# Intel-HLS/GenomicsDB

Measured on AMD Instinct MI355X. Metric: combined-gVCF positions/sec, higher is better.
Workload: dtype u8/int32

## Files before the change

__graft_entry__.py:

```python
import os
import sys

ROOT = os.path.dirname(os.path.abspath(__file__))
sys.path.insert(0, ROOT)
sys.path.insert(0, os.path.join(ROOT, "tests"))


def build():
    from genomicsdb_amd import build as b
    lib = b.build_native(verbose=True)
    b.build_oracle()
    b.build_hostsim()
    b.build_hostsim_variants()
    b.build_hostsim_import()
    b.build_hostsim_inflate()
    b.build_hostsim_import_bcf()
    b.build_hostsim_import_csv()
    b.build_hostsim_dispatch()
    from genomicsdb_amd import synth
    synth.lib()
    import genomicsdb_amd
    from genomicsdb_amd import _lib
    L = _lib.lib()
    for s in _lib.SYMBOLS:
        getattr(L, s)
    print("built", lib)


def smoke():
    import helpers
    from golden_cases import CASES
    import genomicsdb_amd
    case = [c for c in CASES if c[0] == "t6_7_8_vcf_at_0"][0]
    name, callsets, vid, ov, golden, mode = case
    cells = helpers.cells_for(callsets, vid)
    q, pb = helpers.query_json(callsets, vid, ov, mode)
    want, _, _ = helpers.oracle_run(q, cells)
    s = genomicsdb_amd.GenomicsDBQueryStream(query_json=q, cells=cells, buffer_capacity=4096)
    got = s.read()
    s.close()
    assert got == want, "device output differs from the oracle"
    assert got == helpers.golden_text(golden)
    print("smoke ok: %d bytes, bit-exact vs oracle and reference golden" % len(got))


if __name__ == "__main__":
    build()
    if len(sys.argv) > 1 and sys.argv[1] == "smoke":
        smoke()
```

genomicsdb_amd/build.py:

```python
import os
import subprocess
import sys

PKG = os.path.dirname(os.path.abspath(__file__))
ROOT = os.path.dirname(PKG)
CSRC = os.path.join(PKG, "csrc")
OBJ = os.path.join(ROOT, "build", "obj")
LIB = os.path.join(PKG, "libgenomicsdb_amd.so")
TOOL = os.path.join(PKG, "gt_mpi_gather")
TOOLS = {"gt_mpi_gather": TOOL, "vcf2tiledb": os.path.join(PKG, "vcf2tiledb")}

SOURCES = [
    "kernels/gdb_pipeline.hip",
    "kernels/gdb_bgzf.hip",
    "kernels/gdb_import.hip",
    "kernels/gdb_inflate.hip",
    "host/vid_mapper.cc",
    "host/variant_query_config.cc",
    "host/combine_plan.cc",
    "host/fragment.cc",
    "host/reference_genome.cc",
    "host/vcf_importer.cc",
    "host/vcf_index.cc",
    "api/genomicsdb_bcf_generator.cc",
# ... 48 lines not shown
    return LIB


def build_jni(verbose=False):
    jh = os.environ.get("JAVA_HOME", "")
    inc = os.path.join(jh, "include") if jh else ""
    if inc and os.path.exists(os.path.join(inc, "jni.h")):
        incs = ["-I" + inc, "-I" + os.path.join(inc, "linux")]
    else:
        incs = ["-I" + os.path.join(CSRC, "jni", "stub")]
    out = os.path.join(PKG, "libtiledbgenomicsdb.so")
    src = os.path.join(CSRC, "jni", "jni_query_stream.cc")
    if _newer(out, [src, LIB, os.path.join(CSRC, "jni", "stub", "jni.h"), os.path.join(ROOT, "include", "genomicsdb_amd.h")]):
        cmd = ["g++", "-O2", "-std=c++17", "-fPIC", "-shared", "-Wall"] + incs + [src, "-o", out, "-L" + PKG, "-lgenomicsdb_amd", "-Wl,-rpath,$ORIGIN"]
        if verbose:
            print(" ".join(cmd), flush=True)
        subprocess.check_call(cmd)
    return out


def build_oracle():
    subprocess.check_call(["make", "-s", "-C", os.path.join(ROOT, "oracle")])
    return os.path.join(ROOT, "oracle", "liboracle_gvcf.so")


def build_hostsim():
    subprocess.check_call(["make", "-s", "-C", os.path.join(ROOT, "tests", "hostsim")])
    subprocess.check_call(["make", "-s", "-C", os.path.join(ROOT, "tests", "jni_harness")])
    subprocess.check_call(["make", "-s", "-C", os.path.join(ROOT, "tests", "compat")])


def build_hostsim_variants():
    subprocess.check_call(["make", "-s", "-C", os.path.join(ROOT, "tests", "hostsim_variants")])
    return os.path.join(ROOT, "tests", "hostsim_variants", "libhostsim_variants.so")


def build_hostsim_import():
    subprocess.check_call(["make", "-s", "-C", os.path.join(ROOT, "tests", "hostsim_import")])
    return os.path.join(ROOT, "tests", "hostsim_import", "libhostsim_import.so")


def build_hostsim_import_bcf():
    d = os.path.join(ROOT, "tests", "hostsim_import_bcf")
    subprocess.check_call(["make", "-s", "-C", d])
    return os.path.join(d, "libhostsim_import_bcf.so"), os.path.join(d, "malformed_bcf")


def build_hostsim_import_csv():
    d = os.path.join(ROOT, "tests", "hostsim_import_csv")
    subprocess.check_call(["make", "-s", "-C", d])
    return os.path.join(d, "libhostsim_import_csv.so"), os.path.join(d, "hostsim_import_csv_main")


def build_hostsim_inflate():
    subprocess.check_call(["make", "-s", "-C", os.path.join(ROOT, "tests", "hostsim_inflate")])
    return os.path.join(ROOT, "tests", "hostsim_inflate", "libhostsim_inflate.so")


def build_hostsim_dispatch():
    subprocess.check_call(["make", "-s", "-C", os.path.join(ROOT, "tests", "hostsim_dispatch")])
    return os.path.join(ROOT, "tests", "hostsim_dispatch", "libhostsim_dispatch.so")


if __name__ == "__main__":
    print(build_native(verbose=True))
    print(build_oracle())
```

genomicsdb_amd/csrc/core/gdb_core.hpp:

```cpp
#pragma once
#include "gdb_types.h"

#if defined(__HIP_DEVICE_COMPILE__)
#define GDB_FETCH_ADD_U64(p, v) atomicAdd((unsigned long long*)(p), (unsigned long long)(v))
#else
static inline unsigned long long gdb_fetch_add_u64(unsigned long long* p, unsigned long long v) { const unsigned long long o = *p; *p = o + v; return o; }
#define GDB_FETCH_ADD_U64(p, v) gdb_fetch_add_u64((unsigned long long*)(p), (unsigned long long)(v))
#endif

#define GDB_CF_REFBLOCK 1u
#define GDB_CF_DELETION 2u
#define GDB_CF_HAS_NR 4u
#define GDB_CF_HEAVY 8u
#define GDB_CF_IN_WINDOW 16u
#define GDB_CF_NALT(f) (((f) >> 8) & 0xFFu)
#define GDB_CF_PLOIDY(f) (((f) >> 16) & 0xFu)

#define GDB_RF_NON_REF_EXISTS 1u
#define GDB_RF_REMAPPING_NEEDED 2u
#define GDB_RF_SKIP_G_FIELDS 4u

#define GDB_IF_SPANNING 1u
#define GDB_IF_GT_OVERRIDE 2u
#define GDB_IF_NO_NR 4u
// ... 1454 lines not shown
      if (fd.length == GDB_VL_G && (num_merged - 1) > pl.max_diploid_alt_alleles) continue;
      if (fd.ndim == 2) { info_asa_sum(cx, k, f, num_merged, non_ref_exists, !ref_block_only, false, sink, any, err); continue; }
      if (fd.combine_op == GDB_OP_ELEMENT_WISE_SUM || fd.combine_op == GDB_OP_CONCATENATE) {
        if (fd.elem == GDB_ET_FLOAT) info_vector_combine<float>(cx, k, f, fd.combine_op, num_merged, non_ref_exists, !ref_block_only, sink, any, err);
        else info_vector_combine<int32_t>(cx, k, f, fd.combine_op, num_merged, non_ref_exists, !ref_block_only, sink, any, err);
        continue;
      }
      if (fd.elem == GDB_ET_FLOAT) {
        float v;
        if (!reduce_scalar<float>(cx, k, f, fd.combine_op, false, v, err, num_merged, non_ref_exists, !ref_block_only)) continue;
        if (any) sink.put(';');
        sink.write(cx.names.text + cx.names.field_name_off[f], cx.names.field_name_len[f]);
        sink.put('=');
        put_float(sink, v);
      } else {
        int32_t v;
        if (!reduce_scalar<int32_t>(cx, k, f, fd.combine_op, false, v, err, num_merged, non_ref_exists, !ref_block_only)) continue;
        if (any) sink.put(';');
        sink.write(cx.names.text + cx.names.field_name_off[f], cx.names.field_name_len[f]);
        sink.put('=');
        put_i32(sink, v);
      }
      any = true;
    }
    for (int i = 0; i < pl.n_histogram; ++i)
      info_asa_histogram(cx, k, pl.histogram_bin_field[i], pl.histogram_count_field[i], num_merged, non_ref_exists, !ref_block_only, false, sink, any, err);
    int32_t dp = cx.pc.dp_sum[k];
    if ((pl.f_DP >= 0 || pl.f_DP_FORMAT >= 0) && dp > 0 && !ref_block_only) {
      if (any) sink.put(';');
      const char t[] = "DP="; sink.write(t, 3); put_i32(sink, dp);
      any = true;
    }
    if (!any) sink.put('.');
  }
  if (fmt_mask) {
    sink.put('\t');
    bool first = true;
    for (int i = 0; i < pl.n_format; ++i) {
      if (!((fmt_mask >> i) & 1)) continue;
      if (!first) sink.put(':');
      first = false;
      int f = pl.format_field[i];
      if (f == pl.f_DP_FORMAT || f == pl.f_DP) { sink.put('D'); sink.put('P'); }
      else sink.write(cx.names.text + cx.names.field_name_off[f], cx.names.field_name_len[f]);
    }
  }
}

struct EntryCtx {
  FragmentView fr;
  CombinePlan pl;
  CellMeta cm;
  HeavyLists hl;
};
struct RecordInfo { int num_merged; uint32_t rflags; uint32_t fmt_mask; int64_t hbase, hend; };

template <class Sink> GDB_HD void put_int_vector(Sink& s, const int32_t* p, int n) {
  if (n == 0) { s.put('.'); return; }
  for (int j = 0; j < n; ++j) {
    if (p[j] == GDB_BCF_INT32_VECTOR_END) break;
    if (j) s.put(',');
    if (p[j] == GDB_BCF_INT32_MISSING) s.put('.'); else put_i32(s, p[j]);
  }
}
template <class Sink> GDB_HD void put_int_or_missing(Sink& s, bool has, int32_t v) {
  if (!has || v == GDB_BCF_INT32_MISSING) s.put('.'); else put_i32(s, v);
}

struct EntryMaps {
  int8_t* m2i;
  const int8_t* i2m;
  int nr_in;
  int n_in;
  int64_t inc;
  uint32_t cf;
  uint8_t iflag;
  bool remap, nr_exists;
  bool light;
  GDB_HD int lookup(int j) const {
    if (light) return j == 0 ? 0 : nr_in;
    const int v = m2i[j];
    return v >= 0 ? v : nr_in;
  }
};

#define GDB_FIELD_FN GDB_HD

GDB_FIELD_FN int32_t gt_merged_allele(const EntryCtx& cx, const RecordInfo& ri, const EntryMaps& em, int32_t a, int out_i) {
  int32_t m = -1;
  if (em.iflag & GDB_IF_GT_OVERRIDE) {
    const int ra = cx.hl.gt_override[GDB_MAX_PLOIDY * em.inc + (out_i < GDB_MAX_PLOIDY ? out_i : GDB_MAX_PLOIDY - 1)];
    if (ra == 0) m = 0;
    else if (ra == 2) m = ri.num_merged - 1;
    else { for (int q = 1; q < em.n_in; ++q) if (em.i2m && em.i2m[q] >= 0 && em.i2m[q] != ri.num_merged - 1) { m = em.i2m[q]; break; } }
  } else if (a == GDB_TILEDB_NULL_INT32 || a == -1 || a == GDB_BCF_INT32_MISSING) {
    m = -1;
  } else if (!em.remap) {
    m = a;
  } else {
    int8_t mm = -1;
    if (a >= 0 && a < em.n_in) mm = em.i2m ? em.i2m[a] : (a == 0 ? (int8_t)0 : ((em.nr_exists && a == 1) ? (int8_t)(ri.num_merged - 1) : (int8_t)-1));
    if (mm >= 0) m = mm;
    else if ((em.iflag & GDB_IF_SPANNING) && (em.iflag & GDB_IF_NO_NR)) m = -1;
    else m = em.nr_exists ? ri.num_merged - 1 : -1;
  }
  return m;
}
template <class Sink> GDB_FIELD_FN Sink emit_GT(Sink s, const EntryCtx& cx, const RecordInfo& ri, const EntryMaps& em, int64_t c) {
  const CombinePlan& pl = cx.pl;
  const int f = pl.f_GT;
  int n;
  const int32_t* g = cell_field<int32_t>(cx.fr, pl, f, c, n);
  const bool pp = pl.field[f].length == GDB_VL_PP;
  const int step = pp ? 2 : 1;
  int out_i = 0;
  for (int j = 0; j < n; j += step, ++out_i) {
    if (out_i) s.put((pp && g[j - 1] > 0) ? '|' : '/');
    const int32_t m = pl.produce_GT_field ? gt_merged_allele(cx, ri, em, g[j], out_i) : -1;
    if (m < 0) s.put('.'); else put_i32(s, m);
  }
  if (out_i == 0) s.put('.');
  return s;
}

template <class Sink> GDB_FIELD_FN Sink emit_chars(Sink s, const EntryCtx& cx, int f, int64_t c) {
  int n;
  const char* p = cell_field<char>(cx.fr, cx.pl, f, c, n);
  int len = 0;
  while (len < n && p[len]) ++len;
  if (n == 0) s.put('.');
  for (int j = 0; j < len; ++j) { const char ch = p[j]; s.put(ch == 0x07 ? '.' : ch); }
  return s;
}

template <class Sink, class T> GDB_FIELD_FN Sink emit_vector(Sink s, const T* p, int n, uint32_t* err) {
  if (n == 0) { s.put('.'); return s; }
  for (int j = 0; j < n; ++j) {
    if (elem_is_vector_end(p[j])) break;
    if (j) s.put(',');
    put_elem(s, p[j], err);
  }
  return s;
}

template <class Sink, class T> GDB_FIELD_FN Sink emit_remap_alleles(Sink s, const T* p, int n, const EntryMaps& em, int num_merged, bool alt_only, uint32_t* err) {
  const int length = alt_only ? num_merged - 1 : num_merged;
  if (length == 0) { s.put('.'); return s; }
  for (int j = 0; j < length; ++j) {
    if (j) s.put(',');
    const int aj = alt_only ? j + 1 : j;
    const int in_j = em.lookup(aj);
    const int idx = alt_only ? in_j - 1 : in_j;
    const bool has = in_j >= 0 && idx >= 0 && idx < n;
    T v;
    if (has) v = p[idx]; else elem_set_missing(v);
    put_elem(s, v, err);
  }
  return s;
}

template <class Sink, class T> GDB_FIELD_FN Sink emit_remap_genotypes(Sink s, const T* p, int n, const EntryMaps& em, int num_merged, int ploidy, uint32_t* err) {
  if (ploidy == 1) {
    for (int j = 0; j < num_merged; ++j) {
      if (j) s.put(',');
      const int in_j = em.lookup(j);
      const bool has = in_j >= 0 && in_j < n;
      T v;
      if (has) v = p[in_j]; else elem_set_missing(v);
      put_elem(s, v, err);
    }
  } else if (ploidy == 2 && em.light) {
    T v3[3];
    uint64_t w3[3];
    int n3[3];
    const int nr = em.nr_in;
    for (int q = 0; q < 3; ++q) {
      const int gi = q == 0 ? 0 : q == 1 ? (nr >= 0 ? gdb_alleles2gt(0, nr) : -1) : (nr >= 0 ? gdb_alleles2gt(nr, nr) : -1);
      if (gi >= 0 && gi < n) v3[q] = p[gi]; else elem_set_missing(v3[q]);
      n3[q] = elem_pack_text(v3[q], w3[q]);
    }
    for (int kk = 0; kk < num_merged; ++kk)
      for (int j = 0; j <= kk; ++j) {
        const int q = kk == 0 ? 0 : (j == 0 ? 1 : 2);
        if (kk | j) s.put(',');
        if (n3[q]) put_packed(s, w3[q], n3[q]); else put_elem(s, v3[q], err);
      }
  } else if (ploidy == 2) {
    for (int kk = 0; kk < num_merged; ++kk) {
      const int in_k = em.lookup(kk);
      for (int j = 0; j <= kk; ++j) {
        if (kk | j) s.put(',');
        const int in_j = em.lookup(j);
        const bool both = in_j >= 0 && in_k >= 0;
        const int gi = both ? gdb_alleles2gt(in_j, in_k) : 0;
        const bool has = both && gi < n;
        T v;
        if (has) v = p[gi]; else elem_set_missing(v);
        put_elem(s, v, err);
      }
    }
  } else if (ploidy >= 3 && ploidy <= GDB_MAX_PLOIDY) {
    int g[GDB_MAX_PLOIDY], in[GDB_MAX_PLOIDY];
    for (int q = 0; q < ploidy; ++q) g[q] = 0;
    bool first = true;
    do {
      if (!first) s.put(',');
      first = false;
      bool missing = false;
      for (int q = 0; q < ploidy; ++q) { in[q] = em.lookup(g[q]); if (in[q] < 0) missing = true; }
      T v;
      elem_set_missing(v);
      if (!missing) { const int64_t gi = gdb_genotype_index(in, ploidy); if (gi < n) v = p[gi]; }
      put_elem(s, v, err);
    } while (gdb_next_genotype(g, ploidy, num_merged));
  } else {
    *err |= GDB_ERR_UNSUPPORTED_PLOIDY;
    s.put('.');
  }
  return s;
}

GDB_FIELD_FN void build_entry_maps(const EntryCtx& cx, const RecordInfo& ri, int64_t c, EntryMaps& em, int8_t* m2i_store, uint32_t* err) {
  em.m2i = m2i_store;
  em.remap = (ri.rflags & GDB_RF_REMAPPING_NEEDED) != 0;
  em.nr_exists = (ri.rflags & GDB_RF_NON_REF_EXISTS) != 0;
  em.nr_in = -1; em.i2m = nullptr; em.n_in = 0; em.iflag = 0; em.inc = -1; em.cf = 0; em.light = false;
  if (c < 0) return;
  em.cf = cx.cm.cflags[c];
  em.n_in = (int)GDB_CF_NALT(em.cf) + 1;
  if (!em.remap) return;
  if (!(em.cf & GDB_CF_HEAVY)) { em.light = true; em.nr_in = em.nr_exists ? 1 : -1; return; }
  for (int j = 0; j < ri.num_merged; ++j) em.m2i[j] = -1;
  if (em.cf & GDB_CF_HEAVY) {
    const int32_t row = cx.fr.row[c];
    int64_t lo = ri.hbase, hi = ri.hend;
    while (lo < hi) { int64_t mid = (lo + hi) >> 1; if (cx.fr.row[cx.hl.cell[mid]] < row) lo = mid + 1; else hi = mid; }
    if (lo < ri.hend && cx.hl.cell[lo] == c) em.inc = lo; else *err |= GDB_ERR_INTERNAL;
  }
  if (em.inc >= 0) {
    em.i2m = cx.hl.i2m + cx.hl.i2m_off[em.inc];
    em.iflag = cx.hl.iflags[em.inc];
    for (int a = 0; a < em.n_in; ++a) { const int8_t t = em.i2m[a]; if (t >= 0) em.m2i[t] = (int8_t)a; }
    if (em.nr_exists && (em.cf & GDB_CF_HAS_NR) && em.m2i[ri.num_merged - 1] >= 0) em.nr_in = em.m2i[ri.num_merged - 1];
  }
}

template <class Sink> GDB_HD Sink emit_field(Sink s, const EntryCtx& cx, const RecordInfo& ri, const EntryMaps& em, int i, int64_t c, uint32_t* err) {
  const CombinePlan& pl = cx.pl;
  const int f = pl.format_field[i];
  const GdbFieldDesc& fd = pl.field[f];
  if (f == pl.f_DP && pl.f_DP_FORMAT >= 0) {
    int32_t v = GDB_BCF_INT32_MISSING;
    if (field_valid(cx.cm, c, pl.f_DP_FORMAT)) { int n; const int32_t* p = cell_field<int32_t>(cx.fr, pl, pl.f_DP_FORMAT, c, n); if (n > 0) v = p[0]; }
    if (gdb_int_valid(v)) put_i32(s, v); else s.put('.');
  } else if (!field_valid(cx.cm, c, f)) {
    s.put('.');
  } else if (f == pl.f_GT) {
    s = emit_GT(s, cx, ri, em, c);
  } else if (fd.elem == GDB_ET_CHAR || fd.elem == GDB_ET_FLAG) {
    s = emit_chars(s, cx, f, c);
  } else if (fd.elem == GDB_ET_FLOAT) {
    int n;
    const float* p = cell_field<float>(cx.fr, pl, f, c, n);
    const bool allele_dep = fd.length == GDB_VL_A || fd.length == GDB_VL_R || fd.length == GDB_VL_G;
    if (!em.remap || !allele_dep) s = emit_vector(s, p, n, err);
    else if (fd.length == GDB_VL_G) s = emit_remap_genotypes(s, p, n, em, ri.num_merged, (int)GDB_CF_PLOIDY(em.cf), err);
    else s = emit_remap_alleles(s, p, n, em, ri.num_merged, fd.length == GDB_VL_A, err);
  } else if (fd.elem != GDB_ET_INT) {
    *err |= GDB_ERR_INTERNAL;
    s.put('.');
  } else {
    int n;
    const int32_t* p = cell_field<int32_t>(cx.fr, pl, f, c, n);
    const bool allele_dep = fd.length == GDB_VL_A || fd.length == GDB_VL_R || fd.length == GDB_VL_G;
    if (!em.remap || !allele_dep) s = emit_vector(s, p, n, err);
    else if (fd.length == GDB_VL_G) s = emit_remap_genotypes(s, p, n, em, ri.num_merged, (int)GDB_CF_PLOIDY(em.cf), err);
    else s = emit_remap_alleles(s, p, n, em, ri.num_merged, fd.length == GDB_VL_A, err);
  }
  return s;
}

template <class Sink> GDB_HD Sink entry_emit(const EntryCtx& cx, const RecordInfo& ri, int64_t c, Sink s, uint32_t* err) {
  const CombinePlan& pl = cx.pl;
  EntryMaps em;
  int8_t m2i_store[GDB_MAX_MERGED_ALLELES];
  build_entry_maps(cx, ri, c, em, m2i_store, err);
  bool first = true;
  for (int i = 0; i < pl.n_format; ++i) {
    if ((ri.fmt_mask >> i) & 1) {
      if (!first) s.put(':');
      first = false;
      if (c < 0) s.put('.');
      else s = emit_field(s, cx, ri, em, i, c, err);
    }
  }
  return s;
}
```

genomicsdb_amd/csrc/core/gdb_types.h:

```cpp
#pragma once
#include <stdint.h>

#if defined(__HIPCC__)
#define GDB_HD __host__ __device__ __forceinline__
#define GDB_HD_NOINLINE __host__ __device__
#else
#define GDB_HD inline
#define GDB_HD_NOINLINE
#endif

#define GDB_MAX_FIELDS 48
#define GDB_MAX_INFO_FIELDS 24
#define GDB_MAX_FORMAT_FIELDS 24
#define GDB_MAX_MERGED_ALLELES 128
#define GDB_MAX_INPUT_ALLELES 64
#define GDB_MAX_PLOIDY 8
#define GDB_MAX_INFO_VECTOR 64
#define GDB_MAX_ID_TOKENS 16
#define GDB_MAX_FILTER_IDS 16
#define GDB_MAX_PIPELINES_PER_PROCESS 256
#define GDB_MAX_HISTOGRAM_FIELDS 8

#define GDB_BCF_INT32_MISSING ((int32_t)0x80000000)
#define GDB_BCF_INT32_VECTOR_END ((int32_t)0x80000001)
// ... 21 lines not shown
  GDB_ERR_TOO_MANY_ID_TOKENS = 1u << 7,
  GDB_ERR_INFO_VECTOR_TOO_LONG = 1u << 8,
  GDB_ERR_CELL_STREAM = 1u << 9,
  GDB_ERR_TOO_MANY_FILTER_IDS = 1u << 10
};

struct GdbFieldDesc {
  int32_t elem;
  int32_t length;
  int32_t fixed_num;
  int32_t combine_op;
  int32_t is_info, is_format;
  int32_t known_enum;
  int32_t ndim;
  int32_t elem2d;
  int32_t delim0, delim1;
};

struct GdbColumn {
  const void* data;
  const uint32_t* off;
};

struct FragmentView {
  int64_t ncells;
  const int32_t* row;
  const int64_t* begin;
  const int64_t* end;
  GdbColumn col[GDB_MAX_FIELDS];
  int64_t nmarkers;
  const int64_t* marker_begin;
};

struct CombinePlan {
  int32_t nfields;
  GdbFieldDesc field[GDB_MAX_FIELDS];
  int32_t f_REF, f_ALT, f_GT, f_PL, f_DP, f_MIN_DP, f_DP_FORMAT, f_FILTER, f_QUAL, f_ID;
  int32_t n_info;
  int32_t info_field[GDB_MAX_INFO_FIELDS];
  int32_t n_histogram;
  int32_t histogram_bin_field[GDB_MAX_HISTOGRAM_FIELDS], histogram_count_field[GDB_MAX_HISTOGRAM_FIELDS];
  int32_t n_format;
  int32_t format_field[GDB_MAX_FORMAT_FIELDS];
  int32_t produce_GT_field, produce_FILTER_field, sites_only_query, min_PL_GT_for_spanning_deletions;
  int32_t max_diploid_alt_alleles;
  int32_t id_order_unordered_set;
  int32_t qual_combine_op;
  int32_t num_query_rows;
  int32_t bcf_mode;
  int32_t use_missing_values_not_vector_end;
  int32_t bcf_n_sample;
  int32_t bcf_end_id, bcf_dp_id;
  int32_t bcf_id[GDB_MAX_FIELDS];
};

struct GdbContig { int64_t offset, length; int32_t name_off, name_len; int32_t rid, pad; };

struct QueryWindow {
  int64_t qb, qe;
  const int32_t* row_to_qrow;
  int32_t num_array_rows;
  const GdbContig* contigs;
  int32_t ncontigs;
  const char* contig_names;
  const char* ref_bases;
  int64_t ref_begin, ref_len;
};
```

genomicsdb_amd/csrc/host/combine_plan.cc:

```cpp
#include "combine_plan.h"

#include <algorithm>
#include <array>
#include <map>
#include <unordered_map>
#include <cstring>
#include <set>

namespace genomicsdb_amd {

std::string HostPlan::bcf_header_bytes(bool keep_idx_fields) const {
  std::string text;
  for (size_t i = 0; i < header_lines.size(); ++i) {
    const std::string& l = header_lines[i];
    if (keep_idx_fields && header_line_idx[i] >= 0 && !l.empty() && l.back() == '>') text += l.substr(0, l.size() - 1) + ",IDX=" + std::to_string(header_line_idx[i]) + ">";
    else text += l;
    text += '\n';
  }
  text += header_text.substr(header_text.rfind("#CHROM"));
  std::string out("BCF\2\2", 5);
  const uint32_t l_text = (uint32_t)text.size() + 1;
  out.append((const char*)&l_text, 4);
  out += text;
  out.push_back('\0');
// ... 150 lines not shown
        throw UnsupportedOnDeviceException("INFO reducer on non-numeric field " + fi->m_name);
      if (pl.n_info >= GDB_MAX_INFO_FIELDS) throw UnsupportedOnDeviceException("too many INFO fields");
      pl.info_field[pl.n_info++] = f;
      add_field_to_hdr_if_missing(fi->m_vcf_name, 1);
    }
    if (add_FORMAT) {
      if (fi->m_is_vcf_FORMAT_field || op == GDB_OP_MOVE_TO_FORMAT) {
        if (fi->is_length_allele_dependent() && fi->m_element_type != GDB_ET_INT && fi->m_element_type != GDB_ET_FLOAT)
          throw UnsupportedOnDeviceException("allele-dependent non-numeric FORMAT field " + fi->m_name);
        fmt_list.push_back(f);
        add_field_to_hdr_if_missing(fi->m_vcf_name, 2);
      } else {
        dp_info_plan_field = f;
        add_field_to_hdr_if_missing("DP", 1);
      }
    }
  }
  for (auto& kv : histogram_pairs) {
    if (pl.n_histogram >= GDB_MAX_HISTOGRAM_FIELDS) throw UnsupportedOnDeviceException("too many histogram_sum fields");
    if (kv.second[0] < 0 || kv.second[1] < 0)
      throw BroadCombinedGVCFException("histogram_sum needs both tuple elements of field " + vid.get_field_info(kv.first).m_name + " among the queried attributes");
    pl.histogram_bin_field[pl.n_histogram] = kv.second[0];
    pl.histogram_count_field[pl.n_histogram] = kv.second[1];
    ++pl.n_histogram;
  }
  if (pl.f_FILTER >= 0)
    for (unsigned i = 0; i < vid.get_num_fields(); ++i) if (vid.get_field_info(i).m_is_vcf_FILTER_field) add_field_to_hdr_if_missing(vid.get_field_info(i).m_vcf_name, 0);
  if (!sites_only) {
    for (int f : fmt_list) if (f == pl.f_GT) pl.format_field[pl.n_format++] = f;
    for (int f : fmt_list) {
      if (f == pl.f_GT || f == pl.f_DP_FORMAT) continue;
      if (pl.n_format >= GDB_MAX_FORMAT_FIELDS - 1) throw UnsupportedOnDeviceException("too many FORMAT fields");
      pl.format_field[pl.n_format++] = f;
    }
    if (pl.f_DP_FORMAT >= 0 && (dp_info_plan_field >= 0 || std::find(fmt_list.begin(), fmt_list.end(), pl.f_DP_FORMAT) != fmt_list.end()))
      pl.format_field[pl.n_format++] = dp_info_plan_field >= 0 ? dp_info_plan_field : pl.f_DP_FORMAT;
  }
  if (dp_info_plan_field < 0 && pl.f_DP >= 0) {
    pl.f_DP = -1;
  }
  const FieldInfo* qual_info = vid.get_field_info("QUAL");
  if (qual_info && pl.f_QUAL >= 0 && qual_info->m_VCF_field_combine_operation != GDB_OP_UNKNOWN) {
    GdbCombineOp op = qual_info->m_VCF_field_combine_operation;
    if (op != GDB_OP_SUM && op != GDB_OP_MEAN && op != GDB_OP_MEDIAN) throw UnsupportedOnDeviceException("QUAL combine operation");
    pl.qual_combine_op = op;
  }
  pl.produce_GT_field = qc.produce_GT_field();
  pl.produce_FILTER_field = qc.produce_FILTER_field() && pl.f_FILTER >= 0;
  pl.sites_only_query = sites_only;
  pl.min_PL_GT_for_spanning_deletions = qc.produce_GT_with_min_PL_value_for_spanning_deletions();
  pl.max_diploid_alt_alleles = (int)qc.get_max_diploid_alt_alleles_that_can_be_genotyped();
  pl.id_order_unordered_set = qc.id_union_order_unordered_set() ? 1 : 0;
  pl.num_query_rows = (int)qc.get_num_rows_to_query();
  for (unsigned i = 0; i < vid.get_num_contigs(); ++i) {
    const ContigInfo& c = vid.get_contig_info(i);
    if (!hdr_contigs.count(c.m_name)) lines.push_back("##contig=<ID=" + c.m_name + ",length=" + std::to_string(c.m_length) + ">");
    GdbContig g;
    g.offset = c.m_tiledb_column_offset;
    g.length = c.m_length;
    g.name_off = (int32_t)hp.contig_names.size();
    g.name_len = (int32_t)c.m_name.size();
    hp.contig_names += c.m_name;
    hp.contigs.push_back(g);
  }
  {
    std::vector<std::pair<std::string, int>> dict;
    auto find_id = [&](const std::string& id) -> int { for (auto& d : dict) if (d.first == id) return d.second; return -1; };
    dict.push_back(std::make_pair(std::string("PASS"), 0));
    std::vector<std::pair<std::string, int>> ctg_dict;
    for (auto& l : lines) {
      int idx = -1;
      const bool is_dict = l.rfind("##FILTER=", 0) == 0 || l.rfind("##INFO=", 0) == 0 || l.rfind("##FORMAT=", 0) == 0;
      const bool is_ctg = l.rfind("##contig=", 0) == 0;
      size_t idp = l.find("<ID=");
      if ((is_dict || is_ctg) && idp != std::string::npos) {
        size_t ide = l.find_first_of(",>", idp + 4);
        const std::string id = l.substr(idp + 4, ide - idp - 4);
        if (is_dict) { idx = find_id(id); if (idx < 0) { idx = (int)dict.size(); dict.push_back(std::make_pair(id, idx)); } }
        else { idx = (int)ctg_dict.size(); ctg_dict.push_back(std::make_pair(id, idx)); }
      }
      hp.header_lines.push_back(l);
      hp.header_line_idx.push_back(idx);
    }
    for (int f = 0; f < GDB_MAX_FIELDS; ++f) pl.bcf_id[f] = -1;
    for (int f = 0; f < pl.nfields; ++f) { const FieldInfo* fi = vid.get_field_info(hp.field_names[(size_t)f]); if (fi) pl.bcf_id[f] = find_id(fi->m_vcf_name); }
    pl.bcf_end_id = find_id("END");
    pl.bcf_dp_id = find_id("DP");
    for (unsigned i = 0; i < vid.get_num_fields(); ++i) {
      const FieldInfo& fi = vid.get_field_info(i);
      hp.filter_bcf_id.push_back(have[0].count(fi.m_vcf_name) ? find_id(fi.m_vcf_name) : -1);
    }
    for (auto& g : hp.contigs) {
      const std::string name = hp.contig_names.substr((size_t)g.name_off, (size_t)g.name_len);
      g.rid = -1; g.pad = 0;
      for (auto& c : ctg_dict) if (c.first == name) g.rid = c.second;
    }
  }
  pl.bcf_mode = (output_format == "bu" || output_format == "b") ? 1 : 0;
  hp.bgzf = output_format == "z" || output_format == "b";
  if (!(output_format.empty() || output_format == "v" || output_format == "bu" || output_format == "z" || output_format == "b"))
    throw UnsupportedOnDeviceException("VCF output format \"" + output_format + "\": known formats are \"\" (VCF text), \"z\" (BGZF-compressed VCF), \"bu\" (BCF2) and \"b\" (BGZF-compressed BCF2)");
  pl.use_missing_values_not_vector_end = use_missing_values_not_vector_end ? 1 : 0;
  pl.bcf_n_sample = sites_only ? 0 : (int32_t)qc.get_num_rows_to_query();
  if (pl.bcf_mode && pl.bcf_end_id < 0) throw BroadCombinedGVCFException("BCF output needs an INFO END line in the header");
  std::sort(hp.contigs.begin(), hp.contigs.end(), [](const GdbContig& a, const GdbContig& b) { return a.offset < b.offset; });
  for (auto& l : lines) { hp.header_text += l; hp.header_text += '\n'; }
// ... 30 lines not shown
```

genomicsdb_amd/csrc/kernels/gdb_pipeline.hip:

```cpp
#include <hip/hip_runtime.h>

#include <fcntl.h>
#include <sys/stat.h>
#include <unistd.h>
#include <zlib.h>

#include <algorithm>
#include <cstdio>
#include <cstdlib>
#include <chrono>
#include <cstring>
#include <memory>
#include <mutex>
#include <thread>
#include <vector>

#include <rocprim/device/device_radix_sort.hpp>
#include <rocprim/device/device_reduce.hpp>
#include <rocprim/device/device_scan.hpp>
#include <rocprim/iterator/reverse_iterator.hpp>

#include "../core/gdb_stages.hpp"
#include "../core/gdb_bcf.hpp"
#include "../core/gdb_calls.hpp"
// ... 5040 lines not shown
      if ((fd.combine_op == GDB_OP_MEDIAN || fd.combine_op == GDB_OP_SUM || fd.combine_op == GDB_OP_MEAN) && (fd.elem == GDB_ET_FLOAT || fd.elem == GDB_ET_INT) && fd.length != GDB_VL_A)
        fields.push_back(std::make_pair(pl.info_field[i], 0));
    }
    if (pl.qual_combine_op != GDB_OP_UNKNOWN && pl.f_QUAL >= 0) fields.push_back(std::make_pair(pl.f_QUAL, 1));
    if (!fields.empty()) {
      S.scalar_pre.ensure(fields.size() * (size_t)T);
      for (size_t s = 0; s < fields.size(); ++s) {
        hipLaunchKernelGGL(k_scalar_values, dim3(blocks_for(T)), dim3(kBlock), 0, st, fr, pl, cm, rec, (const uint64_t*)S.inc_keys_sorted.p, (const int64_t*)S.inc_vals_sorted.p, T,
                           (int64_t)N, fields[s].first, fields[s].second, S.scalar_pre.p + s * (size_t)T);
        pre.slot[fields[s].first] = (int8_t)s;
      }
      pre.val = S.scalar_pre.p; pre.stride = T; pre.enabled = 1;
    }
  }
  HugeSites huge;
  memset(&huge, 0, sizeof(huge));
  SiteCtx sx0{fr, pl, cm, rec, hl, pc, nt, qw, so, med, big, tie, pre, huge};
  const int32_t huge_threshold = (P > 0 && T / P >= 24 && P <= (int64_t)kMaxHugeRecords) ? 24 : kHugeRecord;
  if (T > (int64_t)huge_threshold && !getenv("GDBAMD_NO_HUGE_SITES")) {
    S.huge_index.ensure((size_t)P); S.huge_list.ensure(kMaxHugeRecords); S.huge_out.ensure(kMaxHugeRecords); S.d_sx0.ensure(1);
    HIP_CHECK(hipMemcpyAsync(S.d_sx0.p, &sx0, sizeof(SiteCtx), hipMemcpyHostToDevice, st));
    STAGE("k_site_huge");
    hipLaunchKernelGGL(k_huge_records, dim3(blocks_for(P)), dim3(kBlock), 0, st, (const int64_t*)S.hbase.p, P, huge_threshold, S.huge_index.p, S.huge_list.p, S.counters.p + 3);
    hipLaunchKernelGGL(k_site_huge, dim3(1024), dim3(kHugeBlock), 0, st, (const SiteCtx*)S.d_sx0.p, (const int32_t*)S.huge_list.p, (const int32_t*)(S.counters.p + 3), S.huge_out.p, S.err.p);
    huge.index = S.huge_index.p; huge.out = S.huge_out.p; huge.enabled = 1;
  }
  SiteCtx sx{fr, pl, cm, rec, hl, pc, nt, qw, so, med, big, tie, pre, huge};
  S.d_sx.ensure(1);
  HIP_CHECK(hipMemcpyAsync(S.d_sx.p, &sx, sizeof(SiteCtx), hipMemcpyHostToDevice, st));
  STAGE("k_site_size");
  S.site_staging.ensure((size_t)P * kSiteStride + 64);
  S.spill_buf.ensure((size_t)P * kSpillTail); S.spill_chunk.ensure((size_t)P);
  const int32_t* site_order = nullptr;
  {
    static const bool sorted_sites = !(getenv("GDBAMD_SITE_ORDER") && atoi(getenv("GDBAMD_SITE_ORDER")) == 0);
    if (sorted_sites && P >= 4096) {
      S.site_key.ensure((size_t)P); S.site_key_sorted.ensure((size_t)P); S.site_ord_in.ensure((size_t)P); S.site_ord.ensure((size_t)P);
      hipLaunchKernelGGL(k_site_order_keys, dim3(blocks_for(P)), dim3(kBlock), 0, st, (const int64_t*)S.hbase.p, P, S.site_key.p, S.site_ord_in.p);
      S.sort_pairs(S.site_key.p, S.site_key_sorted.p, S.site_ord_in.p, S.site_ord.p, (size_t)P, 8);
      site_order = S.site_ord.p;
    }
  }
  hipLaunchKernelGGL(k_site_size, dim3(blocks_for(P, 64)), dim3(64), 0, st, S.d_sx.p, site_order, S.site_staging.p, SpillPool{S.spill_buf.p}, S.spill_chunk.p, S.err.p);
  S.remap_total.ensure(1);
  HIP_CHECK(hipMemsetAsync(S.remap_total.p, 0, sizeof(unsigned long long), st));
  for (int i = 0; i < pl.n_format; ++i)
    if (pl.format_field[i] == pl.f_PL && pl.f_PL >= 0)
      hipLaunchKernelGGL(k_remap_elements, dim3(blocks_for(P)), dim3(kBlock), 0, st, so, (const int32_t*)(d_fmt + (size_t)i * stride), P, i, S.remap_total.p);
  HIP_CHECK(hipEventRecord(ev[2], st));
  const int nchunks = (N + kAsmRows - 1) / kAsmRows;
  const size_t nchunk_total = (size_t)P * nchunks;
  S.chunk_size.ensure(nchunk_total + 1); S.chunk_off.ensure(nchunk_total + 2); S.rec_off.ensure(P + 2);
  RowIndex ri{S.row_ptr.p, S.perm.p, S.rm_begin.p};
  EntryCtx ex{fr, pl, cm, hl};
  HIP_CHECK(hipMemcpyToSymbolAsync(HIP_SYMBOL(c_ex), &ex, sizeof(EntryCtx), (size_t)S.ctx_slot * sizeof(EntryCtx), hipMemcpyHostToDevice, st));
  if (T >= (1ll << 32)) throw GenomicsDBDeviceException("more than 2^32 (record, variant call) incidences in one interval: split the query interval");
  S.type_hkeys.ensure(kTypeHash); S.type_hrep.ensure(kTypeHash); S.type_hid.ensure(kTypeHash); S.type_rep.ensure(kMaxTypes); S.rtype.ensure(P);
  HIP_CHECK(hipMemsetAsync(S.type_hkeys.p, 0xFF, kTypeHash * sizeof(unsigned long long), st));
  HIP_CHECK(hipMemsetAsync(S.type_hrep.p, 0x7F, kTypeHash * sizeof(int32_t), st));
  HIP_CHECK(hipMemsetAsync(S.type_hid.p, 0xFF, kTypeHash, st));
  HIP_CHECK(hipMemsetAsync(S.type_rep.p, 0, kMaxTypes * sizeof(int32_t), st));
  STAGE("k_type_insert");
  hipLaunchKernelGGL(k_type_insert, dim3(blocks_for(P)), dim3(kBlock), 0, st, so, P, S.type_hkeys.p, S.type_hrep.p);
  hipLaunchKernelGGL(k_type_assign, dim3(1), dim3(64), 0, st, S.type_hkeys.p, S.type_hrep.p, max_tabled_types(), S.type_hid.p, S.type_rep.p, S.counters.p + 1);
  S.untabled.ensure(P + 1); S.ubase.ensure(P + 1); S.urec.ensure(P + 1);
  hipLaunchKernelGGL(k_type_lookup, dim3(blocks_for(P)), dim3(kBlock), 0, st, so, P, S.type_hkeys.p, S.type_hid.p, S.rtype.p, S.untabled.p);
  S.excl_scan(S.untabled.p, S.ubase.p, (size_t)P);
  S.tmask.ensure(CW); S.nslots.ensure(CW + 1); S.tbase.ensure(CW + 1);
  STAGE("k_cell_types");
  {
    const size_t nocc = (size_t)kMaxTypes * (size_t)(P + 1);
    S.type_occ.ensure(nocc);
    HIP_CHECK(hipMemsetAsync(S.type_occ.p, 0, nocc * sizeof(uint32_t), st));
    hipLaunchKernelGGL(k_type_onehot, dim3(blocks_for(P)), dim3(kBlock), 0, st, (const uint8_t*)S.rtype.p, P, S.type_occ.p);
    S.excl_scan(S.type_occ.p, S.type_occ.p, nocc);
  }
  hipLaunchKernelGGL(k_cell_types, dim3(blocks_for(CW)), dim3(kBlock), 0, st, S.cflags.p, S.k_lo.p, S.k_hi.p, (const uint32_t*)S.type_occ.p, P,
                     (const int32_t*)(S.counters.p + 1), c_base, CW, S.tmask.p, S.nslots.p);
  S.excl_scan(S.nslots.p, S.tbase.p, (size_t)CW);
  uint32_t ur_a = 0, ur_b = 0, sl_a = 0, sl_b = 0;
  int32_t ntypes = 0;
  S.read_back_many({{&ur_a, S.ubase.p + (P - 1), 4}, {&ur_b, S.untabled.p + (P - 1), 4}, {&sl_a, S.tbase.p + (CW - 1), 4}, {&sl_b, S.nslots.p + (CW - 1), 4},
                    {&ntypes, S.counters.p + 1, 4}});
  const int64_t UR = (int64_t)ur_a + ur_b;
  const uint64_t SL = (uint64_t)sl_a + sl_b;
  if (UR > 0) hipLaunchKernelGGL(k_untabled_records, dim3(blocks_for(P)), dim3(kBlock), 0, st, S.untabled.p, S.ubase.p, P, S.urec.p);
  const uint64_t NS = (uint64_t)kMaxTypes + SL + (uint64_t)T + (uint64_t)UR * (uint64_t)N;
  if (NS >= (1ull << 32)) throw GenomicsDBDeviceException("entry text table exceeds 2^32 slots: split the query interval");
  S.slot_len.ensure(NS + 1); S.slot_units.ensure(NS + 1); S.slot_off.ensure(NS + 1); S.slot_desc.ensure(NS + 1);
  if (NS * (uint64_t)(kSlotStride / 16) >= (uint64_t)kOverflowBit) throw GenomicsDBDeviceException("entry text table exceeds 32 GiB: split the query interval");
  S.pool.ensure((size_t)NS * kSlotStride + 64);
  S.slot_bump.ensure(kBumpShards * 4);
  HIP_CHECK(hipMemsetAsync(S.slot_bump.p, 0, kBumpShards * 4 * sizeof(unsigned int), st));
  S.slot_over.ensure(kBumpShards);
  HIP_CHECK(hipMemsetAsync(S.slot_over.p, 0, kBumpShards * sizeof(unsigned int), st));
  bool wide = S.long_texts_seen;
  if (const char* e = getenv("GDBAMD_SLOT_STRIP")) wide = atoi(e) >= 256;
  auto shard_units_of = [&](size_t cap_bytes) { return (uint32_t)std::min<uint64_t>((uint64_t)(cap_bytes > 64 ? (cap_bytes - 64) / 16 : 0) / kBumpShards, ((uint64_t)kOverflowBit - 1) / kBumpShards); };
  if (wide) S.pool_ovf.ensure(std::max<size_t>((size_t)kBumpShards * ((size_t)S.pool_ovf_need * 16 + ((size_t)S.pool_ovf_need * 16 >> 3)), (size_t)1 << 20) + 64);
  SlotTable stt{S.slot_len.p, S.slot_off.p, S.pool.p, S.pool_ovf.p, (uint32_t)kMaxTypes, (uint32_t)(kMaxTypes + SL), (uint32_t)(kMaxTypes + SL + (uint64_t)T), S.slot_off.p, S.slot_bump.p,
                wide ? shard_units_of(S.pool_ovf.cap) : 0u, (int32_t)S.ctx_slot, pl.bcf_mode, pl.bcf_mode ? (uint32_t)kSlotStride : (uint32_t)kInlineText,
                (const int64_t*)S.hoff.p, (const int32_t*)S.k_lo.p, c_base, S.slot_over.p};
  STAGE("k_slots<0>");
#define GDB_SLOT_KERNELS(PASSN, W) do { \
  hipLaunchKernelGGL((k_slots_nocall<PASSN, W>), dim3(1), dim3(kMaxTypes), 0, st, stt, so, S.type_rep.p, ntypes, S.err.p); \
  if (SL > 0) hipLaunchKernelGGL((k_slots_light<PASSN, W>), dim3(blocks_for((int64_t)SL, light_block<W>())), dim3(light_block<W>()), 0, st, stt, so, S.type_rep.p, S.tmask.p, S.tbase.p, (const uint32_t*)S.slot_cell.p, c_base, (int64_t)SL, slot_regroup() ? 1 : 0, S.err.p); \
  if (T > 0) hipLaunchKernelGGL((k_slots_heavy<PASSN, W>), dim3(blocks_for(T, 64)), dim3(64), 0, st, stt, so, S.inc_keys_sorted.p, S.inc_vals_sorted.p, T, (int64_t)N, S.err.p); \
// ... 344 lines not shown
```

Measured before the change: 39.64 million.

## Add light-path per-cell FORMAT emitter driven by precomputed per-field op codes

```diff
diff --git a/__graft_entry__.py b/__graft_entry__.py
--- a/__graft_entry__.py
+++ b/__graft_entry__.py
@@ -17,6 +17,7 @@
     b.build_hostsim_import_bcf()
     b.build_hostsim_import_csv()
     b.build_hostsim_dispatch()
+    b.build_hostsim_light_emit()
     from genomicsdb_amd import synth
     synth.lib()
     import genomicsdb_amd
diff --git a/genomicsdb_amd/build.py b/genomicsdb_amd/build.py
--- a/genomicsdb_amd/build.py
+++ b/genomicsdb_amd/build.py
@@ -124,6 +124,12 @@
     return os.path.join(d, "libhostsim_import_csv.so"), os.path.join(d, "hostsim_import_csv_main")
 
 
+def build_hostsim_light_emit():
+    d = os.path.join(ROOT, "tests", "hostsim_light_emit")
+    subprocess.check_call(["make", "-s", "-C", d])
+    return os.path.join(d, "light_emit_diff"), os.path.join(d, "light_emit_diff_san")
+
+
 def build_hostsim_inflate():
     subprocess.check_call(["make", "-s", "-C", os.path.join(ROOT, "tests", "hostsim_inflate")])
     return os.path.join(ROOT, "tests", "hostsim_inflate", "libhostsim_inflate.so")
diff --git a/genomicsdb_amd/csrc/core/gdb_core.hpp b/genomicsdb_amd/csrc/core/gdb_core.hpp
--- a/genomicsdb_amd/csrc/core/gdb_core.hpp
+++ b/genomicsdb_amd/csrc/core/gdb_core.hpp
@@ -1530,6 +1530,7 @@
   CombinePlan pl;
   CellMeta cm;
   HeavyLists hl;
+  uint32_t generic_emit;
 };
 struct RecordInfo { int num_merged; uint32_t rflags; uint32_t fmt_mask; int64_t hbase, hend; };
 
@@ -1625,13 +1626,14 @@
   const int length = alt_only ? num_merged - 1 : num_merged;
   if (length == 0) { s.put('.'); return s; }
   for (int j = 0; j < length; ++j) {
-    if (j) s.put(',');
     const int aj = alt_only ? j + 1 : j;
     const int in_j = em.lookup(aj);
     const int idx = alt_only ? in_j - 1 : in_j;
     const bool has = in_j >= 0 && idx >= 0 && idx < n;
     T v;
     if (has) v = p[idx]; else elem_set_missing(v);
+    if (elem_is_vector_end(v)) break;
+    if (j) s.put(',');
     put_elem(s, v, err);
   }
   return s;
@@ -1640,11 +1642,12 @@
 template <class Sink, class T> GDB_FIELD_FN Sink emit_remap_genotypes(Sink s, const T* p, int n, const EntryMaps& em, int num_merged, int ploidy, uint32_t* err) {
   if (ploidy == 1) {
     for (int j = 0; j < num_merged; ++j) {
-      if (j) s.put(',');
       const int in_j = em.lookup(j);
       const bool has = in_j >= 0 && in_j < n;
       T v;
       if (has) v = p[in_j]; else elem_set_missing(v);
+      if (elem_is_vector_end(v)) break;
+      if (j) s.put(',');
       put_elem(s, v, err);
     }
   } else if (ploidy == 2 && em.light) {
@@ -1660,6 +1663,7 @@
     for (int kk = 0; kk < num_merged; ++kk)
       for (int j = 0; j <= kk; ++j) {
         const int q = kk == 0 ? 0 : (j == 0 ? 1 : 2);
+        if (elem_is_vector_end(v3[q])) return s;
         if (kk | j) s.put(',');
         if (n3[q]) put_packed(s, w3[q], n3[q]); else put_elem(s, v3[q], err);
       }
@@ -1667,13 +1671,14 @@
     for (int kk = 0; kk < num_merged; ++kk) {
       const int in_k = em.lookup(kk);
       for (int j = 0; j <= kk; ++j) {
-        if (kk | j) s.put(',');
         const int in_j = em.lookup(j);
         const bool both = in_j >= 0 && in_k >= 0;
         const int gi = both ? gdb_alleles2gt(in_j, in_k) : 0;
         const bool has = both && gi < n;
         T v;
         if (has) v = p[gi]; else elem_set_missing(v);
+        if (elem_is_vector_end(v)) return s;
+        if (kk | j) s.put(',');
         put_elem(s, v, err);
       }
     }
@@ -1682,13 +1687,14 @@
     for (int q = 0; q < ploidy; ++q) g[q] = 0;
     bool first = true;
     do {
-      if (!first) s.put(',');
-      first = false;
       bool missing = false;
       for (int q = 0; q < ploidy; ++q) { in[q] = em.lookup(g[q]); if (in[q] < 0) missing = true; }
       T v;
       elem_set_missing(v);
       if (!missing) { const int64_t gi = gdb_genotype_index(in, ploidy); if (gi < n) v = p[gi]; }
+      if (elem_is_vector_end(v)) break;
+      if (!first) s.put(',');
+      first = false;
       put_elem(s, v, err);
     } while (gdb_next_genotype(g, ploidy, num_merged));
   } else {
@@ -1730,7 +1736,7 @@
   if (f == pl.f_DP && pl.f_DP_FORMAT >= 0) {
     int32_t v = GDB_BCF_INT32_MISSING;
     if (field_valid(cx.cm, c, pl.f_DP_FORMAT)) { int n; const int32_t* p = cell_field<int32_t>(cx.fr, pl, pl.f_DP_FORMAT, c, n); if (n > 0) v = p[0]; }
-    if (gdb_int_valid(v)) put_i32(s, v); else s.put('.');
+    if (gdb_int_valid(v)) put_i32(s, v); else if (v != GDB_BCF_INT32_VECTOR_END) s.put('.');
   } else if (!field_valid(cx.cm, c, f)) {
     s.put('.');
   } else if (f == pl.f_GT) {
@@ -1758,8 +1764,133 @@
   return s;
 }
 
+GDB_HD int light_token(uint32_t sep, int32_t v, uint64_t& w) {
+  int n;
+  if (v == GDB_BCF_INT32_MISSING) { w = (uint64_t)'.'; n = 1; }
+  else if ((uint32_t)v < 100u) {
+    const uint32_t q = (uint32_t)v / 10u, r = (uint32_t)v - q * 10u;
+    w = q ? (uint64_t)(('0' + q) | (('0' + r) << 8)) : (uint64_t)('0' + r);
+    n = q ? 2 : 1;
+  }
+  else if ((uint32_t)v < 10000000u) w = gdb_pack_digits((uint32_t)v, n);
+  else return 0;
+  if (sep) { w = (w << 8) | (uint64_t)sep; ++n; }
+  return n;
+}
+template <class Sink> GDB_HD void put_token_w(Sink& s, uint64_t w, int n, uint32_t sep, int32_t v) {
+  if (n) put_packed(s, w, n);
+  else { if (sep) s.put((char)sep); put_i32(s, v); }
+}
+template <class Sink> GDB_HD void put_token(Sink& s, uint32_t sep, int32_t v) {
+  uint64_t w = 0;
+  const int n = light_token(sep, v, w);
+  put_token_w(s, w, n, sep, v);
+}
+template <class Sink> GDB_HD Sink entry_emit_light(const EntryCtx& cx, const RecordInfo& ri, int64_t c, uint32_t cf, uint64_t vmask, Sink s, uint32_t* err) {
+  const CombinePlan& pl = cx.pl;
+  const bool remap = (ri.rflags & GDB_RF_REMAPPING_NEEDED) != 0, nr_exists = (ri.rflags & GDB_RF_NON_REF_EXISTS) != 0;
+  const int nm = ri.num_merged;
+  const int nr_in = nr_exists ? 1 : -1;
+  uint32_t next_sep = 0;
+  for (int i = 0; i < pl.n_format; ++i) {
+    if (!((ri.fmt_mask >> i) & 1u)) continue;
+    const uint32_t sep = next_sep;
+    next_sep = ':';
+    const uint32_t op = pl.light_op[i];
+    const int f = (int)(op & 0xFFu);
+    uint32_t kind = (op >> 8) & 0xFu;
+    if (!((vmask >> f) & 1ull)) { put_token(s, sep, GDB_BCF_INT32_MISSING); continue; }
+    const GdbColumn& col = cx.fr.col[f];
+    int n;
+    const int32_t* p;
+    if (col.off) { const uint32_t a = col.off[c], b = col.off[c + 1]; n = (int)(b - a); p = (const int32_t*)col.data + a; }
+    else { n = (int)(op >> 12); p = (const int32_t*)col.data + c * n; }
+    if (kind >= GDB_LOP_R) {
+      if (!remap) kind = GDB_LOP_VEC;
+      else if (kind == GDB_LOP_G && GDB_CF_PLOIDY(cf) == 1u) kind = GDB_LOP_R;
+    }
+    switch (kind) {
+      case GDB_LOP_FIRST: {
+        const int32_t v = n > 0 ? p[0] : GDB_BCF_INT32_MISSING;
+        if (v != GDB_BCF_INT32_VECTOR_END) put_token(s, sep, v); else if (sep) s.put((char)sep);
+      } break;
+      case GDB_LOP_GT: case GDB_LOP_GT_PP: {
+        const bool pp = kind == GDB_LOP_GT_PP;
+        int out_i = 0;
+        for (int j = 0; j < n; j += pp ? 2 : 1, ++out_i) {
+          const uint32_t sp = out_i ? ((pp && p[j - 1] > 0) ? (uint32_t)'|' : (uint32_t)'/') : sep;
+          const int32_t a = p[j];
+          int32_t mg = GDB_BCF_INT32_MISSING;
+          if (pl.produce_GT_field && a != GDB_TILEDB_NULL_INT32 && a != -1 && a != GDB_BCF_INT32_MISSING) {
+            if (!remap) mg = a < 0 ? GDB_BCF_INT32_MISSING : a;
+            else mg = a == 0 ? 0 : (nr_exists ? nm - 1 : GDB_BCF_INT32_MISSING);
+          }
+          put_token(s, sp, mg);
+        }
+        if (out_i == 0) put_token(s, sep, GDB_BCF_INT32_MISSING);
+      } break;
+      case GDB_LOP_VEC: {
+        if (n == 0) { put_token(s, sep, GDB_BCF_INT32_MISSING); break; }
+        int j = 0;
+        for (; j < n; ++j) {
+          const int32_t v = p[j];
+          if (v == GDB_BCF_INT32_VECTOR_END) break;
+          put_token(s, j ? (uint32_t)',' : sep, v);
+        }
+        if (j == 0 && sep) s.put((char)sep);
+      } break;
+      case GDB_LOP_R: {
+        if (nm <= 0) { put_token(s, sep, GDB_BCF_INT32_MISSING); break; }
+        const int32_t v0 = n > 0 ? p[0] : GDB_BCF_INT32_MISSING, v1 = nr_in >= 0 && nr_in < n ? p[nr_in] : GDB_BCF_INT32_MISSING;
+        if (v0 == GDB_BCF_INT32_VECTOR_END) { if (sep) s.put((char)sep); break; }
+        put_token(s, sep, v0);
+        if (v1 == GDB_BCF_INT32_VECTOR_END) break;
+        uint64_t w1 = 0;
+        const int n1 = light_token(',', v1, w1);
+        for (int j = 1; j < nm; ++j) put_token_w(s, w1, n1, ',', v1);
+      } break;
+      case GDB_LOP_A: {
+        if (nm <= 1) { put_token(s, sep, GDB_BCF_INT32_MISSING); break; }
+        const int32_t v = nr_in >= 0 && nr_in - 1 < n ? p[nr_in - 1] : GDB_BCF_INT32_MISSING;
+        if (v == GDB_BCF_INT32_VECTOR_END) { if (sep) s.put((char)sep); break; }
+        put_token(s, sep, v);
+        uint64_t w1 = 0;
+        const int n1 = light_token(',', v, w1);
+        for (int j = 2; j < nm; ++j) put_token_w(s, w1, n1, ',', v);
+      } break;
+      case GDB_LOP_G: {
+        if (GDB_CF_PLOIDY(cf) != 2u) { *err |= GDB_ERR_UNSUPPORTED_PLOIDY; put_token(s, sep, GDB_BCF_INT32_MISSING); break; }
+        if (nm <= 0) { put_token(s, sep, GDB_BCF_INT32_MISSING); break; }
+        const int32_t v0 = n > 0 ? p[0] : GDB_BCF_INT32_MISSING;
+        const int32_t v1 = nr_exists && n > 1 ? p[1] : GDB_BCF_INT32_MISSING, v2 = nr_exists && n > 2 ? p[2] : GDB_BCF_INT32_MISSING;
+        if (v0 == GDB_BCF_INT32_VECTOR_END) { if (sep) s.put((char)sep); break; }
+        put_token(s, sep, v0);
+        if (nm < 2 || v1 == GDB_BCF_INT32_VECTOR_END) break;
+        uint64_t w1 = 0, w2 = 0;
+        const int n1 = light_token(',', v1, w1), n2 = light_token(',', v2, w2);
+        put_token_w(s, w1, n1, ',', v1);
+        if (v2 == GDB_BCF_INT32_VECTOR_END) break;
+        put_token_w(s, w2, n2, ',', v2);
+        for (int kk = 2; kk < nm; ++kk) {
+          put_token_w(s, w1, n1, ',', v1);
+          for (int j = 1; j <= kk; ++j) put_token_w(s, w2, n2, ',', v2);
+        }
+      } break;
+      default: *err |= GDB_ERR_INTERNAL; put_token(s, sep, GDB_BCF_INT32_MISSING); break;
+    }
+  }
+  return s;
+}
+
 template <class Sink> GDB_HD Sink entry_emit(const EntryCtx& cx, const RecordInfo& ri, int64_t c, Sink s, uint32_t* err) {
   const CombinePlan& pl = cx.pl;
+  if (c >= 0 && pl.light_ready && !cx.generic_emit) {
+    const uint32_t cf = cx.cm.cflags[c];
+    const uint64_t vmask = cx.cm.vmask[c];
+    const uint64_t slow = (uint64_t)pl.light_slow_lo | ((uint64_t)pl.light_slow_hi << 32);
+    if ((!(cf & GDB_CF_HEAVY) || !(ri.rflags & GDB_RF_REMAPPING_NEEDED)) && GDB_CF_PLOIDY(cf) <= 2u && !(vmask & slow))
+      return entry_emit_light(cx, ri, c, cf, vmask, s, err);
+  }
   EntryMaps em;
   int8_t m2i_store[GDB_MAX_MERGED_ALLELES];
   build_entry_maps(cx, ri, c, em, m2i_store, err);
diff --git a/genomicsdb_amd/csrc/core/gdb_types.h b/genomicsdb_amd/csrc/core/gdb_types.h
--- a/genomicsdb_amd/csrc/core/gdb_types.h
+++ b/genomicsdb_amd/csrc/core/gdb_types.h
@@ -97,7 +97,30 @@
   int32_t bcf_n_sample;
   int32_t bcf_end_id, bcf_dp_id;
   int32_t bcf_id[GDB_MAX_FIELDS];
+  int32_t light_ready;
+  uint32_t light_op[GDB_MAX_FORMAT_FIELDS];
+  uint32_t light_slow_lo, light_slow_hi;
 };
+enum GdbLightOp { GDB_LOP_FIRST = 1, GDB_LOP_GT, GDB_LOP_GT_PP, GDB_LOP_VEC, GDB_LOP_R, GDB_LOP_A, GDB_LOP_G };
+inline void gdb_build_light_ops(CombinePlan& pl) {
+  uint64_t slow = 0;
+  for (int i = 0; i < pl.n_format && i < GDB_MAX_FORMAT_FIELDS; ++i) {
+    const int f = pl.format_field[i];
+    const bool dp_rule = f == pl.f_DP && pl.f_DP_FORMAT >= 0;
+    const int fr = dp_rule ? pl.f_DP_FORMAT : f;
+    const GdbFieldDesc& fd = pl.field[fr];
+    uint32_t kind;
+    if (dp_rule) kind = GDB_LOP_FIRST;
+    else if (f == pl.f_GT) kind = fd.length == GDB_VL_PP ? GDB_LOP_GT_PP : GDB_LOP_GT;
+    else kind = fd.length == GDB_VL_R ? GDB_LOP_R : fd.length == GDB_VL_A ? GDB_LOP_A : fd.length == GDB_VL_G ? GDB_LOP_G : GDB_LOP_VEC;
+    const bool fits = fd.fixed_num >= 0 && fd.fixed_num < (1 << 20);
+    if (fd.elem != GDB_ET_INT || !fits) slow |= 1ull << fr;
+    pl.light_op[i] = (uint32_t)fr | (kind << 8) | ((fits ? (uint32_t)fd.fixed_num : 0u) << 12);
+  }
+  pl.light_slow_lo = (uint32_t)slow;
+  pl.light_slow_hi = (uint32_t)(slow >> 32);
+  pl.light_ready = 1;
+}
 
 struct GdbContig { int64_t offset, length; int32_t name_off, name_len; int32_t rid, pad; };
 
diff --git a/genomicsdb_amd/csrc/host/combine_plan.cc b/genomicsdb_amd/csrc/host/combine_plan.cc
--- a/genomicsdb_amd/csrc/host/combine_plan.cc
+++ b/genomicsdb_amd/csrc/host/combine_plan.cc
@@ -226,6 +226,7 @@
   pl.max_diploid_alt_alleles = (int)qc.get_max_diploid_alt_alleles_that_can_be_genotyped();
   pl.id_order_unordered_set = qc.id_union_order_unordered_set() ? 1 : 0;
   pl.num_query_rows = (int)qc.get_num_rows_to_query();
+  gdb_build_light_ops(pl);
   for (unsigned i = 0; i < vid.get_num_contigs(); ++i) {
     const ContigInfo& c = vid.get_contig_info(i);
     if (!hdr_contigs.count(c.m_name)) lines.push_back("##contig=<ID=" + c.m_name + ",length=" + std::to_string(c.m_length) + ">");
diff --git a/genomicsdb_amd/csrc/kernels/gdb_pipeline.hip b/genomicsdb_amd/csrc/kernels/gdb_pipeline.hip
--- a/genomicsdb_amd/csrc/kernels/gdb_pipeline.hip
+++ b/genomicsdb_amd/csrc/kernels/gdb_pipeline.hip
@@ -5116,7 +5116,8 @@
   const size_t nchunk_total = (size_t)P * nchunks;
   S.chunk_size.ensure(nchunk_total + 1); S.chunk_off.ensure(nchunk_total + 2); S.rec_off.ensure(P + 2);
   RowIndex ri{S.row_ptr.p, S.perm.p, S.rm_begin.p};
-  EntryCtx ex{fr, pl, cm, hl};
+  EntryCtx ex{fr, pl, cm, hl, 0u};
+  if (const char* e = getenv("GDBAMD_LIGHT_EMIT")) ex.generic_emit = *e == '0' ? 1u : 0u;
   HIP_CHECK(hipMemcpyToSymbolAsync(HIP_SYMBOL(c_ex), &ex, sizeof(EntryCtx), (size_t)S.ctx_slot * sizeof(EntryCtx), hipMemcpyHostToDevice, st));
   if (T >= (1ll << 32)) throw GenomicsDBDeviceException("more than 2^32 (record, variant call) incidences in one interval: split the query interval");
   S.type_hkeys.ensure(kTypeHash); S.type_hrep.ensure(kTypeHash); S.type_hid.ensure(kTypeHash); S.type_rep.ensure(kMaxTypes); S.rtype.ensure(P);
```

Result: no change. 40.37 million (median of 6 runs) (+1.8%).
